# luisdamiano/sparseRGPs

Hardware: AMD Instinct MI355X
Metric: sparse-GP objective+gradient evals/sec at n=1e6, m=1024, d=8 (higher is better)
Workload: dtype f64; 1 GPU; C3: Titsias VI ELBO + gradient, n=1000000, m=1024, d=8, ard, P=10, knots fixed; n=1000000, m=1024, d=8, kernel=ard, parallelism=single

## Files before the change

sparsergps_amd/csrc/capi.hip:

```cpp
#include <math.h>

#include <cmath>
#include <stdarg.h>
#include <stdio.h>
#include <stdlib.h>
#include <string.h>
#include <time.h>

#include <algorithm>
#include <string>
#include <vector>

#include "../../include/sgp.h"
#include "../../include/sgp_diag.h"
#include "sgp_internal.h"

#ifdef SGP_HOST_PROBE
extern "C" __attribute__((visibility("default"))) double sgp_probe_t[4] = {0.0, 0.0, 0.0, 0.0};
#endif
#include "sgp_probe.h"
#include "sgp_multi.h"

namespace {

// ... 246 lines not shown
  bool lap_expo_rows = false;
  const double* lap_av = nullptr;
  int lap_family = SGP_FAM_POISSON;
  std::vector<double> lap_objs;
  bool timing = false;
  std::string timing_only;
  int64_t timing_evals = 0;
  std::vector<Timer> timers;
  std::vector<hipEvent_t> pool;
  size_t pool_used = 0;
};

namespace {

constexpr int SC_LD22 = 0, SC_LDB = 1, SC_TU = 2, SC_TRKS = 3, SC_TRBS = 4, SC_RR = 5,
              SC_G22 = 16;
constexpr int SC_N = 64;
constexpr int SLAB_SMALL = 1024 * (SGP_MAXD + 2);
constexpr int KNOT_PART_ROWS = 256;
constexpr int RB_N = 256;

constexpr int RB_SEGS = SGP_RB_SEGS;

#ifdef SGP_HOST_PROBE
static double hp_now() {
  struct timespec ts;
  clock_gettime(CLOCK_MONOTONIC, &ts);
  return (double)ts.tv_sec + 1e-9 * (double)ts.tv_nsec;
}
static double hp_t0 = 0.0, hp_issue = 0.0, hp_wait = 0.0, hp_tail = 0.0, hp_prev_end = 0.0,
              hp_gap = 0.0;
static long hp_n = 0;
// ... 512 lines not shown
                   hipSuccess && cus > 0)
      c->sk_slots = 2 * cus;
    if (c->sk_slots > 0) {
      st = st ? st : dalloc(&c->sk_ws, sgp_con_sk_doubles(c->sk_slots));
      st = st ? st : dalloc(&c->sk_flags, c->sk_slots + 1);
      if (!st && hipMemset(c->sk_flags, 0, sizeof(unsigned) * (c->sk_slots + 1)) != hipSuccess) {
        set_err("hipMemset of the contraction hand-over flags failed");
        st = SGP_EHIP;
      }
    }
  }
  c->slab_small_cap = std::max<int64_t>(SLAB_SMALL, mp * (SGP_MAXD + 2));
  st = st ? st : dalloc(&c->slab_small, c->slab_small_cap);
  st = st ? st : dalloc(&c->slab_aux, c->slab_small_cap);
  st = st ? st : dalloc(&c->rr_dev, 1);
  st = st ? st : dalloc(&c->mmpart, mp);
  st = st ? st : dalloc(&c->sc, SC_N);
  st = st ? st : dalloc(&c->y, np_);
  st = st ? st : dalloc(&c->mu, np_);
  st = st ? st : dalloc(&c->tslab, (np_ / 64) * mp);
  st = st ? st : dalloc(&c->khash, mp);
  st = st ? st : dalloc(&c->kidx, mp);
  st = st ? st : dalloc(&c->cflag, np_);
  if (!st && (hipHostMalloc(reinterpret_cast<void**>(&c->pin),
                            sizeof(double) * (mp * d + m_max + (m_max + 1) / 2 + 8 + RB_N),
                            hipHostMallocDefault) != hipSuccess ||
              hipEventCreateWithFlags(&c->ev_pin, hipEventDisableTiming) != hipSuccess)) {
    set_err("pinned staging allocation failed");
    st = SGP_ENOMEM;
  }
  if (st) {
// ... 212 lines not shown
  }
  c->pack_red1 = enable != 0;
  return SGP_OK;
}

static int64_t vi_red1_toff(const sgp_ctx* c, int64_t mp) {
  return c->pack_red1 ? syrk_packed_doubles(mp) : mp * mp;
}

int64_t sgp_knot_red_extra(int d, int64_t m) { return round_up(m, SGP_TILE) * d; }

static int contract_pass(sgp_ctx* c, const double* M, ConArgs ca, double* rec_out,
                         double* knot_out, bool knot_acc) {
  int64_t nrec = 0, nwg = 0;
  if (c->knot_on) ca.knot_slab = c->knot_slab;
  const bool fused = ca.uvec != nullptr && ca.alpha_in == nullptr;
  if (fused) ca.alpha_out = c->alpha;
  if (c->sk_ws) {
    if (++c->sk_epoch == 0) ++c->sk_epoch;
    ca.sk_ws = c->sk_ws;
    ca.sk_flags = c->sk_flags;
    ca.sk_epoch = c->sk_epoch;
    ca.sk_slots = c->sk_slots;
    ca.sk_status = c->status + 3;
    ca.sk_dp = con_sk_dp();
  }
  HIPCHK(launch_contract_args(c->kp, c->K, M, c->X, c->n_pad, c->n, c->n_pad, c->U, c->mp, c->m,
                              c->mp, ca, c->slab_con, &nrec, &nwg, c->stream));
  const bool flags_known = c->cflag_gen == c->knots_gen;
  HIPCHK(launch_records(c->slab_con, nrec, nwg, c->X, c->n_pad, c->n, c->kp.d, c->U, c->mp, c->m,
                        c->khash, c->kidx, c->K, c->mp, M, ca, fused ? c->alpha : ca.alpha_in,
                        c->slab_small, c->slab_small_cap, 1 + c->kp.L, rec_out, c->cflag,
                        flags_known ? 2 : 1, c->stream, c->defer_rec ? &c->rec_defer : nullptr));
  c->cflag_gen = c->knots_gen;
  if (c->knot_on)
    HIPCHK(launch_knot_reduce(c->knot_slab, c->n_pad / SGP_TILE, c->mp, c->kp.d, c->knot_part,
                              KNOT_PART_ROWS * c->mp_max * c->d,
                              knot_out, knot_acc, c->stream));
  return SGP_OK;
}

static int knot_finish(sgp_ctx* c, const double* knot_red, const double* uvec, const double* Ainv,
                       const double* Binv, const double* M3, double a, double b, double cc,
                       const double* v, const double* w, double e2) {
  if (!c->knot_on) return SGP_OK;
  const KernParams& kp = c->kp;
// ... 253 lines not shown
    Scope tm(c, "mm_vectors");
    const bool k22_via_t = c->t_deferred;
    if (c->t_deferred) {
      HIPCHK(hipStreamWaitEvent(c->stream, c->ev_t, 0));
      c->t_deferred = false;
    }
    if (flags & SGP_FLAG_OBJ_ONLY) {
      HIPCHK(dense_gemv(c->Binv, mp, t, 1.0 / z, c->uvec, c->stream));
      HIPCHK(launch_dot(t, c->uvec, mp, c->slab_small, c->sc + SC_TU, c->stream));
      HIPCHK(hipMemcpyAsync(c->sc + SC_RR, red1 + toff + mp, sizeof(double),
                            hipMemcpyDeviceToDevice, c->stream));
      HIPCHK(hipStreamWaitEvent(c->stream, c->ev_m3, 0));
      c->phase = 2;
      return SGP_OK;
    }
    if (!k22_via_t) HIPCHK(hipStreamWaitEvent(c->stream, c->ev_k22, 0));
    HIPCHK(launch_vi_mm_rows(c->Binv, c->K22inv, S, t, mp, 1.0 / z, 1.0 / kp.tau2, -1.0 / z,
                             c->uvec, c->Pm, c->mmpart, c->stream));
    HIPCHK(hipEventRecord(c->ev_bm, c->stream));
  }
  {
    HIPCHK(hipStreamWaitEvent(c->aux_lo, c->ev_bm, 0));
    HIPCHK(launch_vi_mm_scalars(t, c->uvec, c->mmpart, mp, red1 + toff + mp, c->sc + SC_TU,
                                c->sc + SC_TRBS, c->sc + SC_RR, c->aux_lo));
    HIPCHK(launch_sum_small(c->logdB, mp / SGP_DB, c->sc + SC_LDB, c->aux_lo));
    Scope tm(c, "contract_kmm", c->aux_lo);
    int nb = 0;
    HIPCHK(launch_contract_kmm(kp, c->U, c->mp, c->m, mp, c->uvec, c->K22inv, c->Binv, c->M3,
                               -0.5, 0.5, -1.0 / (2.0 * kp.tau2), nullptr, nullptr, 0.0,
                               c->slab_aux, c->slab_small_cap, &nb, c->aux_lo));
    HIPCHK(launch_colsum(c->slab_aux, nb, kp.P, c->sc + SC_G22, c->aux_lo));
    HIPCHK(hipEventRecord(c->ev_m3, c->aux_lo));
  }
  {
    Scope tm(c, "contract_knm");
    ConArgs ca;
    ca.r = c->r;
    ca.invz = 1.0 / z;
    ca.uvec = c->uvec;
    ca.cdiag = c->cdiag;
    ca.count_a2 = 1;
    int st2 = contract_pass(c, c->Pm, ca, red2, red2 + sgp_vi_red2_count(kp.kernel, kp.d), false);
    if (st2) return st2;
  }
  HIPCHK(hipStreamWaitEvent(c->stream, c->ev_m3, 0));
  c->phase = 2;
  return SGP_OK;
}

int sgp_vi_finish(sgp_ctx* c, const double* red2, double* obj, double* grad) {
  MULTI_REFUSE(c, "sgp_vi_finish");
  const bool obj_only = c && (c->flags & SGP_FLAG_OBJ_ONLY);
  if (!c || !red2 || !obj || (!grad && !obj_only)) {
    set_err("invalid arguments");
    return SGP_EINVAL;
  }
  if (c->phase != 2) { set_err("sgp_vi_finish called before sgp_vi_phase2"); return SGP_EINVAL; }
  {
    const hipError_t e = hipSetDevice(c->device);
// ... 32 lines not shown
    fprintf(stderr, "\n");
  }
  const double n = (double)c->n_global;
  const double z = kp.tau2 + c->delta;
  const double ld22 = 2.0 * sc[SC_LD22], ldB = 2.0 * sc[SC_LDB];
  const double rr = sc[SC_RR], tu = sc[SC_TU], trKS = sc[SC_TRKS], trBS = sc[SC_TRBS];
  const double quad = -0.5 * rr / z + 0.5 * tu / z;
  const double logdet22 = (c->flags & SGP_FLAG_R_DET) ? log(exp(ld22)) : ld22;
  const double det_part = -0.5 * (n * log(z) - logdet22 + ldB);
  const double trace_term = -(1.0 / (2.0 * kp.tau2)) * (n * (kp.sig2 + c->delta) - trKS);
  *obj = quad + det_part - (n / 2.0) * log(2.0 * M_PI) + trace_term;
  if (obj_only) {
    c->knot_raw.clear();
    return SGP_OK;
  }
  const double e_sig = r2[0];
  const double c_sum = r2[1 + L], c_cnt = r2[2 + L], c_dg = r2[3 + L], aTa = r2[4 + L];
  const double trSinv = n / z - trBS / (z * z);
  const double trW = 0.5 * (aTa - trSinv);
  grad[0] = 2.0 * e_sig + sc[SC_G22] - n * kp.sig2 / kp.tau2;
  for (int q = 0; q < L; ++q) grad[1 + q] = r2[1 + q] + sc[SC_G22 + 1 + q];
  grad[L + 1] = 2.0 * kp.tau2 * (c_sum - (c_cnt - c->delta * c_dg) / kp.tau2) +
                2.0 * kp.tau2 * trW - 2.0 * trace_term;
  return knot_finish(c, red2 + n2, c->uvec, c->K22inv, c->Binv, c->M3, -0.5, 0.5,
                     -1.0 / (2.0 * kp.tau2), nullptr, nullptr, 0.0);
}

int sgp_eval_vi(sgp_ctx* c, int kernel, const double* theta, const double* U, int64_t m,
                int64_t ldu, double delta, unsigned flags, double* obj, double* grad) {
  MULTI_FWD(c, obj && (grad || (flags & SGP_FLAG_OBJ_ONLY)) ? multi_eval_vi(c->multi, kernel, theta, U, m, ldu, delta, flags, obj, grad) : multi_bad_args());
  if (!c) { set_err("context is NULL"); return SGP_EINVAL; }
  if (!obj || (!grad && !(flags & SGP_FLAG_OBJ_ONLY))) {
    set_err("obj is NULL, or grad is NULL without SGP_FLAG_OBJ_ONLY");
    return SGP_EINVAL;
  }
#ifdef SGP_HOST_PROBE
// ... 1430 lines not shown
```

sparsergps_amd/csrc/k_dense.hip:

```cpp
#include <stdlib.h>

#include <atomic>

#include "sgp_internal.h"
#include "sgp_probe.h"

namespace {

__device__ __forceinline__ double wave_sum(double v) {
#pragma unroll
  for (int o = 32; o > 0; o >>= 1) v += __shfl_xor(v, o, 64);
  return v;
}

__device__ __forceinline__ double block_sum(double v, double* sh) {
  const int lane = threadIdx.x & 63, w = threadIdx.x >> 6;
  v = wave_sum(v);
  if (lane == 0) sh[w] = v;
  __syncthreads();
  double t = 0.0;
  const int nw = blockDim.x >> 6;
  for (int q = 0; q < nw; ++q) t += sh[q];
  __syncthreads();
  return t;
// ... 760 lines not shown
                                                    int64_t n_pad, double* __restrict__ omega,
                                                    double* __restrict__ slab) {
  __shared__ double sh[4];
  double s = 0.0;
  for (int64_t i = (int64_t)blockIdx.x * 256 + threadIdx.x; i < n_pad; i += (int64_t)gridDim.x * 256) {
    double o = 0.0;
    if (i < n) o = alpha[i] * alpha[i] - (w[i] - w[i] * w[i] * p[i]);
    omega[i] = o;
    s += o;
  }
  s = block_sum(s, sh);
  if (threadIdx.x == 0) slab[blockIdx.x] = s;
}

__global__ void __launch_bounds__(256) k_vi_mm_rows(const double* __restrict__ Binv,
                                                    const double* __restrict__ K22inv,
                                                    const double* __restrict__ S,
                                                    const double* __restrict__ t, int64_t mp,
                                                    double invz, double a, double b,
                                                    double* __restrict__ u,
                                                    double* __restrict__ P,
                                                    double* __restrict__ part) {
  const int64_t row = (int64_t)blockIdx.x * 4 + (threadIdx.x >> 6);
  const int lane = threadIdx.x & 63;
  if (row >= mp) return;
  const int64_t o = row * mp;
  double su = 0.0, sp = 0.0;
  for (int64_t j = lane; j < mp; j += 64) {
    const double bv = Binv[o + j];
    su = fma(bv, t[j], su);
    sp = fma(bv, S[o + j], sp);
    P[o + j] = a * K22inv[o + j] + b * bv;
  }
  su = wave_sum(su);
  sp = wave_sum(sp);
  if (lane == 0) {
    u[row] = invz * su;
    part[row] = sp;
  }
}

__global__ void __launch_bounds__(256) k_vi_mm_scalars(const double* __restrict__ t,
                                                       const double* __restrict__ u,
                                                       const double* __restrict__ part,
                                                       int64_t mp, const double* __restrict__ rr,
                                                       double* __restrict__ tu_out,
                                                       double* __restrict__ trbs_out,
                                                       double* __restrict__ rr_out) {
  __shared__ double sh[4];
  double a = 0.0, c = 0.0;
  for (int64_t j = threadIdx.x; j < mp; j += 256) {
    a = fma(t[j], u[j], a);
    c += part[j];
  }
  a = block_sum(a, sh);
  c = block_sum(c, sh);
  if (threadIdx.x == 0) {
    *tu_out = a;
    *trbs_out = c;
    *rr_out = *rr;
  }
}

}

hipError_t launch_vi_mm_rows(const double* Binv, const double* K22inv, const double* S,
                             const double* t, int64_t mp, double invz, double a, double b,
                             double* u, double* P, double* part, hipStream_t s) {
  hipLaunchKernelGGL(k_vi_mm_rows, dim3((unsigned)((mp + 3) / 4)), dim3(256), 0, s, Binv, K22inv,
                     S, t, mp, invz, a, b, u, P, part);
  return hipGetLastError();
}

hipError_t launch_vi_mm_scalars(const double* t, const double* u, const double* part, int64_t mp,
                                const double* rr, double* tu_out, double* trbs_out,
                                double* rr_out, hipStream_t s) {
  hipLaunchKernelGGL(k_vi_mm_scalars, dim3(1), dim3(256), 0, s, t, u, part, mp, rr, tu_out,
                     trbs_out, rr_out);
  return hipGetLastError();
}

hipError_t launch_fitc_z(const double* q, int64_t n, int64_t n_pad, double c0, double* w,
                         double* slab, int* nblocks, hipStream_t s) {
  int nb = (int)((n_pad + 255) / 256);
  if (nb > 1024) nb = 1024;
// ... 163 lines not shown
```

sparsergps_amd/csrc/k_mfma.hip:

```cpp
#include <algorithm>
#include <vector>

#include "sgp_internal.h"
#include "sgp_probe.h"

namespace {

constexpr int T128 = 128;
constexpr int BK = 16;
constexpr int SB = 144;
constexpr int SA = 17;
constexpr int SYRK_RGRP = 16;

__device__ __forceinline__ double wave_sum(double v) {
#pragma unroll
  for (int o = 32; o > 0; o >>= 1) v += __shfl_xor(v, o, 64);
  return v;
}

__device__ __forceinline__ int64_t xcd_remap(int64_t orig, int64_t nwg) {
  const int64_t x = orig % 8, q = nwg / 8, r = nwg % 8;
  const int64_t base = (x < r) ? x * (q + 1) : r * (q + 1) + (x - r) * q;
  return base + orig / 8;
}
// ... 763 lines not shown
enum { CON_FULL = 0, CON_TAIL = 1, CON_HEAD = 2 };
constexpr int64_t CON_SK_SLOT = 65 * 256;
struct ConSK {
  double* ws = nullptr;
  int dp = -1;
  unsigned* flags = nullptr;
  unsigned epoch = 0;
  int64_t slot = 0;
  int* status = nullptr;
};

__device__ __forceinline__ unsigned con_ldu_sc1(const unsigned* p) {
  return __hip_atomic_load(p, __ATOMIC_RELAXED, __HIP_MEMORY_SCOPE_AGENT);
}

template <int DT, int EPI, bool V2, bool KNOT, bool FROM_T, bool KU, bool T2, int SKM>
__device__ __forceinline__ void con_tile(
    const KernParams& kp, const double* __restrict__ K, const double* __restrict__ M,
    const double* __restrict__ X, int64_t ldx, int64_t n, int64_t n_pad,
    const double* __restrict__ U, int64_t ldu, int64_t m, int64_t mp, const ConArgs& ca,
    double* __restrict__ slab, int nrec, double* __restrict__ rowq, int64_t ti, int64_t tj,
    int64_t wgid, int kb, int ke, double* lds, double (*red)[SGP_MAXD + 5], double (*s_uk)[BK],
    const ConSK& sk, int part, int tid_in) {
  const double* __restrict__ r = ca.r;
  const double* __restrict__ uvec = ca.uvec;
  const double* __restrict__ cdiag = ca.cdiag;
  constexpr int A_SZ = CON_A_SZ, B_SZ = CON_B_SZ;
  const int64_t ntj = mp / T128;
  const int64_t nwg = (n_pad / T128) * ntj;
  const int64_t i0 = ti * T128, j0 = tj * T128;

  const int tid = tid_in, lane = tid & 63, wv = tid >> 6;
  const int wr = wv >> 1, wc = wv & 1;
  const bool with_u = KU && (uvec != nullptr) && (ca.alpha_in == nullptr);
  constexpr bool with_v = V2;

  d4 acc[4][4];
#pragma unroll
  for (int a = 0; a < 4; ++a)
#pragma unroll
    for (int b = 0; b < 4; ++b) acc[a][b] = d4{0.0, 0.0, 0.0, 0.0};

  const int arow = tid >> 1, acol = (tid & 1) * 8;
  const double2* gA = reinterpret_cast<const double2*>(K + (i0 + arow) * mp + acol);
  const int bk = tid >> 4, bc = tid & 15;
  const double2* gB = reinterpret_cast<const double2*>(M + (int64_t)bk * mp + j0) + bc;
  const int64_t bstep = BK * mp / 2;
  double2 va0, va1, va2, va3, vb0, vb1, vb2, vb3;
  double ku = 0.0, vuk = 0.0;
  const double* __restrict__ uk_src = with_u ? uvec : M;
// ... 121 lines not shown
  SGP_PROBE_CON_SKIP_EPILOGUE()
  double* s_alpha = lds;
  double* s_rs = s_alpha + T128;
  double* s_u = s_rs + T128;
  double* s_cd = s_u + T128;
  double* s_beta = s_cd + T128;
  double* s_v = s_beta + T128;
  double* s_xs = s_v + T128;
  double* s_us = s_xs + T128 * 16;
  double* s_rs2 = lds + 8320;
  static_assert(8320 + T128 <= 2 * (A_SZ + B_SZ), "s_rs2 fits the LDS image");
  ku += __shfl_xor(ku, 1, 64);
  double a2 = 0.0;
  if ((tid & 1) == 0) {
    const int64_t i = i0 + arow;
    const double iz = ca.invz_vec ? ca.invz_vec[i] : ca.invz;
    const double al = ca.alpha_in ? ca.alpha_in[i]
                                  : (with_u ? (r[i] - ku) * iz : 0.0);
    const bool iv = i < n;
    s_alpha[arow] = iv ? al : 0.0;
    s_rs[arow] = iv ? (ca.rs_vec ? ca.rs * ca.rs_vec[i] : ca.rs) : 0.0;
    if constexpr (T2) s_rs2[arow] = iv ? (ca.rs_vec2 ? ca.rs2 * ca.rs_vec2[i] : ca.rs2) : 0.0;
    s_beta[arow] = (with_v && iv) ? ca.beta_in[i] : 0.0;
    if (tj == 0) {
      if (ca.count_a2 && i < n) a2 = al * al;
      if (ca.alpha_out) ca.alpha_out[i] = al;
    }
  }
  const double* Kt = K + i0 * mp + j0;

  if constexpr (EPI == EPI_ROWQUAD) {
    if (ca.tstore != nullptr) {
#pragma unroll
      for (int fm = 0; fm < 4; ++fm)
#pragma unroll
        for (int fn = 0; fn < 4; ++fn)
#pragma unroll
          for (int q = 0; q < 4; ++q)
            ca.tstore[(i0 + wr * 64 + fm * 16 + (lane >> 4) + 4 * q) * mp + j0 + wc * 64 +
                      fn * 16 + (lane & 15)] = acc[fm][fn][q];
    }
// ... 126 lines not shown
          for (int fn = 0; fn < 4; ++fn) {
            const int col = wc * 64 + fn * 16 + (lane & 15);
            double kv[2];
#pragma unroll
            for (int r2 = 0; r2 < 2; ++r2) kv[r2] = kb[(wr * 8 + (lane >> 4) + 4 * r2) * KST + col];
#pragma unroll
            for (int r2 = 0; r2 < 2; ++r2) {
              const int q = 2 * h + r2;
              const int row = wr * 64 + fm * 16 + (lane >> 4) + 4 * q;
              double G = s_rs[row] * acc[fm][fn][q];
              if constexpr (T2) G = fma(s_rs2[row], t2c[r2][fn], G);
              if constexpr (V2) G = fma(s_beta[row], vcol[fn], G);
              G = fma(s_alpha[row], ucol[fn], G);
              double w = G * kv[r2];
              if constexpr ((V2 && KNOT) || FROM_T) w = (j0 + col < m && i0 + row < n) ? w : 0.0;
              Cc[fn] += w;
              acc[fm][fn][q] = w;
            }
          }
#pragma unroll
          for (int r2 = 0; r2 < 2; ++r2)
#pragma unroll
            for (int fn = 0; fn < 4; ++fn)
#ifndef SGP_CON_PROBE_NO_EPI_MFMA
              P[fn] = __builtin_amdgcn_mfma_f64_16x16x4f64(acc[fm][fn][2 * h + r2], xb[r2], P[fn],
                                                           0, 0, 0);
#else
              P[fn][r2] = fma(acc[fm][fn][2 * h + r2], xb[r2], P[fn][r2]);
#endif
          if (hs == 1) SGP_PROBE_CON_STAMP(3);
        }
// ... 18 lines not shown
#pragma unroll
            for (int r4 = 0; r4 < 4; ++r4)
              xb[r4] = s_xs[(wr * 64 + fm * 16 + 4 * r4 + (lane >> 4)) * 16 + (lane & 15)];
#pragma unroll
            for (int r4 = 0; r4 < 4; ++r4)
#pragma unroll
              for (int fn = 0; fn < 4; ++fn)
                P[fn] = __builtin_amdgcn_mfma_f64_16x16x4f64(acc[fm][fn][r4], xb[r4], P[fn], 0,
                                                             0, 0);
          }
        }
        const bool cok = 8 * ch + cc < d;
        double E = 0.0;
#pragma unroll
        for (int fn = 0; fn < 4; ++fn) {
          double C = Cc[fn];
          C += __shfl_xor(C, 16, 64);
          C += __shfl_xor(C, 32, 64);
          if (ch == 0 && (lane >> 4) == 0) e_sig += C;
#pragma unroll
          for (int q = 0; q < 4; ++q) {
            const int jl = wc * 64 + fn * 16 + (lane >> 4) + 4 * q;
            const double Cq = __shfl(C, (lane >> 4) + 4 * q, 64);
            const double u = cok ? s_us[jl * sus + cc] : 0.0;
            const double pv = P[fn][q];
            E += (cp >= 8) ? pv : u * fma(u, Cq, -2.0 * pv);
            if constexpr (KNOT) {
              if (cp < 8) s_kn[(wr * T128 + jl) * 8 + cc] = pv - u * Cq;
            }
          }
        }
        E += __shfl_xor(E, 8, 64);
        E += __shfl_xor(E, 16, 64);
        E += __shfl_xor(E, 32, 64);
        if (ard) {
          if (lane < 8 && 8 * ch + lane < d) red[wv][1 + 8 * ch + lane] = E;
        } else {
          double t = E;
          t += __shfl_xor(t, 1, 64);
          t += __shfl_xor(t, 2, 64);
          t += __shfl_xor(t, 4, 64);
          e_sq += t;
        }
        if constexpr (KNOT) {
          __syncthreads();
          for (int e = tid; e < T128 * 8; e += 256) {
            const int col = e >> 3, c = e & 7, cg = 8 * ch + c;
            if (cg < d)
              ca.knot_slab[(ti * mp + j0 + col) * d + cg] =
                  s_kn[col * 8 + c] + s_kn[(T128 + col) * 8 + c];
          }
        }
      }
#undef CON_XSTAGE
    }

    SGP_PROBE_CON_STAMP(6);
    double v;
    v = wave_sum(e_sig);
    if (lane == 0) red[wv][0] = v;
    if (!ard && lane == 0) red[wv][1] = e_sq * rl2s;
    v = wave_sum(a2);
    if (lane == 0) {
      red[wv][1 + L] = 0.0;
      red[wv][2 + L] = 0.0;
      red[wv][3 + L] = 0.0;
      red[wv][4 + L] = v;
    }
    __syncthreads();
    if (tid < nrec)
      slab[tid * nwg + wgid] = red[0][tid] + red[1][tid] + red[2][tid] + red[3][tid];
    SGP_PROBE_CON_STAMP(2);
  }
  if constexpr (SGP_CON_EPI_PRIO > 0) __builtin_amdgcn_s_setprio(0);
}

template <int DT, int EPI, bool V2 = false, bool KNOT = false, bool FROM_T = false, bool KU = true,
          bool T2 = false>
__global__ void __launch_bounds__(256, 2)
k_contract(KernParams kp, const double* __restrict__ K, const double* __restrict__ M,
           const double* __restrict__ X, int64_t ldx, int64_t n, int64_t n_pad,
           const double* __restrict__ U, int64_t ldu, int64_t m, int64_t mp, ConArgs ca,
           double* __restrict__ slab, int nrec, double* __restrict__ rowq) {
  __shared__ __attribute__((aligned(16))) double lds[CON_LDS];
  __shared__ double red[4][SGP_MAXD + 5];
  __shared__ double s_uk[2][BK];
  const int64_t ntj = mp / T128;
  const int64_t nwg = (n_pad / T128) * ntj;
  const int64_t wgid = xcd_remap(blockIdx.x, nwg);
  con_tile<DT, EPI, V2, KNOT, FROM_T, KU, T2, 0>(
      kp, K, M, X, ldx, n, n_pad, U, ldu, m, mp, ca, slab, nrec, rowq, wgid / ntj, wgid % ntj,
      wgid, 0, (int)(mp / BK), lds, red, s_uk, ConSK{}, CON_FULL, (int)threadIdx.x);
}

template <int DT, bool KNOT>
__global__ void __launch_bounds__(256, 2)
k_contract_sk(KernParams kp, const double* __restrict__ K, const double* __restrict__ M,
              const double* __restrict__ X, int64_t ldx, int64_t n, int64_t n_pad,
              const double* __restrict__ U, int64_t ldu, int64_t m, int64_t mp, ConArgs ca,
              double* __restrict__ slab, int nrec, ConSK sk) {
  __shared__ __attribute__((aligned(16))) double lds[CON_LDS];
  __shared__ double red[4][SGP_MAXD + 5];
  __shared__ double s_uk[2][BK];
  const int64_t ntj = mp / T128;
  const int64_t ntiles = (n_pad / T128) * ntj;
  const int S = (int)(mp / BK);
  const int64_t G = gridDim.x, v = xcd_remap(blockIdx.x, G);
  const int64_t dp_rounds = (sk.dp >= 0 && sk.dp < ntiles / G) ? sk.dp : ntiles / G - 1;
  const int64_t t0 = dp_rounds * G;
  const int64_t Usk = (ntiles - t0) * S;
  const int64_t u1 = Usk * (v + 1) / G;
  int64_t u = Usk * v / G;
  if (u % S != 0) {
    const int64_t tile = t0 + u / S;
    const int kb = (int)(u % S);
    ConSK p = sk;
    p.slot = v;
    con_tile<DT, EPI_GRAD, false, KNOT, false, true, false, CON_TAIL>(
        kp, K, M, X, ldx, n, n_pad, U, ldu, m, mp, ca, slab, nrec, nullptr, tile / ntj,
        tile % ntj, tile, kb, S, lds, red, s_uk, p, CON_TAIL, (int)threadIdx.x);
    u += S - kb;
    __syncthreads();
  }
  int64_t r = 0;
  for (;;) {
    int64_t tile;
    int ke;
    if (r < dp_rounds) {
      tile = r * G + v;
      ke = S;
      ++r;
    } else if (u < u1) {
      tile = t0 + u / S;
      ke = (int)((u1 - u) < (int64_t)S ? (u1 - u) : S);
      u += ke;
    } else {
      break;
    }
    ConSK p = sk;
    p.slot = v + 1;
    int tid;
    asm volatile("v_mov_b32 %0, %1" : "=v"(tid) : "v"((int)threadIdx.x));
    con_tile<DT, EPI_GRAD, false, KNOT, false, true, false, CON_HEAD>(
        kp, K, M, X, ldx, n, n_pad, U, ldu, m, mp, ca, slab, nrec, nullptr, tile / ntj,
        tile % ntj, tile, 0, ke, lds, red, s_uk, p, ke < S ? CON_HEAD : CON_FULL, tid);
    __syncthreads();
  }
}

__global__ void __launch_bounds__(256)
k_knot_reduce1(const double* __restrict__ slab, int64_t ntiles, int64_t ncol,
               double* __restrict__ part) {
  const int64_t col = (int64_t)blockIdx.x * 256 + threadIdx.x;
  const int64_t r = blockIdx.y, G = gridDim.y;
  if (col >= ncol) return;
  double s0 = 0.0, s1 = 0.0, s2 = 0.0, s3 = 0.0;
  int64_t t = r;
  for (; t + 3 * G < ntiles; t += 4 * G) {
// ... 40 lines not shown
      h *= 1099511628211ull;
    }
  }
  return h;
}

struct CoincArgs {
  const double* X; int64_t ldx, n; int d;
  const double* U; int64_t ldu, m;
  const uint64_t* khash; const int* kidx;
  const double* K; int64_t mp; const double* M;
  const double* alpha; const double* uvec; const double* beta; const double* vvec;
  const double* rs_vec; double rs; const double* cdiag;
  uint8_t* cflag; int flag_mode;
  const double* M2; const double* rs_vec2; double rs2;
};

__device__ __forceinline__ void coinc_body(const CoincArgs& ca, int64_t bid, int64_t nblk,
                                           double* __restrict__ part) {
  const double* __restrict__ X = ca.X;
  const double* __restrict__ U = ca.U;
  const double* __restrict__ K = ca.K;
  const double* __restrict__ M = ca.M;
  const int64_t ldx = ca.ldx, n = ca.n, ldu = ca.ldu, m = ca.m, mp = ca.mp;
  const int d = ca.d, flag_mode = ca.flag_mode;
  const uint64_t* __restrict__ khash = ca.khash;
  const int* __restrict__ kidx = ca.kidx;
  const double *alpha = ca.alpha, *uvec = ca.uvec, *beta = ca.beta, *vvec = ca.vvec;
  const double *rs_vec = ca.rs_vec, *cdiag = ca.cdiag;
  const double rs = ca.rs;
// ... 11 lines not shown
    for (int64_t p = lo; p < m && khash[p] == h; ++p) {
      const int64_t j = kidx[p];
      bool eq = true;
      for (int c = 0; c < d; ++c) eq = eq && (X[i + c * ldx] == U[j + c * ldu]);
      if (!eq) continue;
      any = true;
      double t = 0.0;
      for (int64_t k = 0; k < m; ++k) t = fma(K[i * mp + k], M[k * mp + j], t);
      double g = (rs_vec ? rs * rs_vec[i] : rs) * t;
      if (ca.M2) {
        double t2 = 0.0;
        for (int64_t k = 0; k < m; ++k) t2 = fma(K[i * mp + k], ca.M2[k * mp + j], t2);
        g = fma(ca.rs_vec2 ? ca.rs2 * ca.rs_vec2[i] : ca.rs2, t2, g);
      }
      if (beta) g = fma(beta[i], vvec[j], g);
      if (alpha && uvec) g = fma(alpha[i], uvec[j], g);
      a[0] += g;
      a[1] += 1.0;
      a[2] += cdiag ? cdiag[j] : 0.0;
    }
    if (flag_mode == 1) cflag[i] = any ? 1 : 0;
  }
  __shared__ double sh[4][3];
  const int lane = threadIdx.x & 63, w = threadIdx.x >> 6;
  for (int k = 0; k < 3; ++k) {
    const double v = wave_sum(a[k]);
    if (lane == 0) sh[w][k] = v;
  }
  __syncthreads();
  if (threadIdx.x < 3)
    part[bid * 3 + threadIdx.x] =
// ... 507 lines not shown
                          int64_t ldx, int64_t n, int d, const double* U, int64_t ldu, int64_t m,
                          const uint64_t* khash, const int* kidx, const double* K, int64_t mp,
                          const double* M, const ConArgs& cg, const double* alpha, double* part,
                          int64_t part_cap, int coff, double* rec, uint8_t* cflag, int flag_mode,
                          hipStream_t s, RecPass2* defer) {
  if (nrow <= 0 || nrow > 256 || coff < 0 || coff + 3 > nrow) return hipErrorInvalidValue;
  const int G = 32;
  int64_t nbc = (n + 255) / 256;
  if (nbc > 1024) nbc = 1024;
  if (nbc < 1) nbc = 1;
  if (nrow * G + 3 * nbc > part_cap) return hipErrorInvalidValue;
  double* part_r = part;
  double* part_c = part + nrow * G;
  CoincArgs ca{X, ldx, n, d, U, ldu, m, khash, kidx, K, mp, M, alpha, cg.uvec, cg.beta_in,
               cg.vvec, cg.rs_vec, cg.rs, cg.cdiag, cflag, flag_mode, cg.M2, cg.rs_vec2,
               cg.rs2};
  hipLaunchKernelGGL(k_rec_pass1, dim3((unsigned)(nbc + nrow * G)), dim3(256), 0, s, ca,
                     (int)nbc, slab, len, G, part_r, part_c);
  RecPass2 p2;
  p2.part_r = part_r;
  p2.part_c = part_c;
  p2.rec = rec;
  p2.G = G;
  p2.nrow = (int)nrow;
  p2.nbc = (int)nbc;
  p2.coff = coff;
  if (defer != nullptr) *defer = p2;
  else hipLaunchKernelGGL(k_rec_pass2, dim3(1), dim3(256), 0, s, p2);
  return hipGetLastError();
}

// ... 23 lines not shown
}

template <int DT, bool KNOT = false>
static void launch_con_grad(bool v2, const KernParams& kp, const double* K, const double* M,
                            const double* X, int64_t ldx, int64_t n, int64_t n_pad,
                            const double* U, int64_t ldu, int64_t m, int64_t mp,
                            const ConArgs& ca, double* slab, int nrec, int64_t nwg,
                            hipStream_t s) {
  if (!v2 && con_use_sk(ca, nwg, mp)) {
    ConSK sk;
    sk.ws = ca.sk_ws;
    sk.flags = ca.sk_flags;
    sk.epoch = ca.sk_epoch;
    sk.status = ca.sk_status;
    sk.dp = ca.sk_dp;
    hipLaunchKernelGGL((k_contract_sk<DT, KNOT>), dim3((unsigned)ca.sk_slots), dim3(256), 0, s,
                       kp, K, M, X, ldx, n, n_pad, U, ldu, m, mp, ca, slab, nrec, sk);
    return;
  }
  if (v2)
    hipLaunchKernelGGL((k_contract<DT, EPI_GRAD, true, KNOT>), dim3((unsigned)nwg), dim3(256), SGP_CON_SHMEM,
                       s, kp, K, M, X, ldx, n, n_pad, U, ldu, m, mp, ca, slab, nrec,
                       (double*)nullptr);
  else
    hipLaunchKernelGGL((k_contract<DT, EPI_GRAD, false, KNOT>), dim3((unsigned)nwg), dim3(256), SGP_CON_SHMEM,
                       s, kp, K, M, X, ldx, n, n_pad, U, ldu, m, mp, ca, slab, nrec,
                       (double*)nullptr);
}

template <int DT, bool T2>
static void launch_con_from_t2(bool v2, bool kn, const KernParams& kp, const double* K,
                               const double* M, const double* X, int64_t ldx, int64_t n,
                               int64_t n_pad, const double* U, int64_t ldu, int64_t m, int64_t mp,
                               const ConArgs& ca, double* slab, int nrec, int64_t nwg,
                               hipStream_t s) {
// ... 29 lines not shown
                                  nrec, nwg, s);
}

int64_t sgp_con_sk_doubles(int slots) { return (int64_t)(slots + 1) * CON_SK_SLOT; }

hipError_t launch_contract_args(const KernParams& kp, const double* K, const double* M,
                                const double* X, int64_t ldx, int64_t n, int64_t n_pad,
                                const double* U, int64_t ldu, int64_t m, int64_t mp,
                                const ConArgs& ca, double* slab, int64_t* nrec_out,
                                int64_t* nwg_out, hipStream_t s) {
  const int64_t nwg = (n_pad / T128) * (mp / T128);
  const int nrec = kp.L + 5;
  *nrec_out = nrec;
  *nwg_out = nwg;
  if ((ca.tin2 != nullptr) != (ca.M2 != nullptr) || (ca.tin2 && (!ca.tin || kp.d > 8)))
    return hipErrorInvalidValue;
  if (ca.tin != nullptr) {
    if (ca.uvec != nullptr && ca.alpha_in == nullptr) return hipErrorInvalidValue;
    const bool v2 = ca.beta_in != nullptr, kn = ca.knot_slab != nullptr;
    if (kp.d <= 8) launch_con_from_t<8>(v2, kn, kp, K, M, X, ldx, n, n_pad, U, ldu, m, mp, ca, slab,
                                        nrec, nwg, s);
    else launch_con_from_t<SGP_MAXD>(v2, kn, kp, K, M, X, ldx, n, n_pad, U, ldu, m, mp, ca, slab,
                                     nrec, nwg, s);
    return hipGetLastError();
  }
  if (ca.knot_slab != nullptr) {
    const bool v2 = ca.beta_in != nullptr;
    if (kp.d <= 8) launch_con_grad<8, true>(v2, kp, K, M, X, ldx, n, n_pad, U, ldu, m, mp, ca,
                                            slab, nrec, nwg, s);
    else launch_con_grad<SGP_MAXD, true>(v2, kp, K, M, X, ldx, n, n_pad, U, ldu, m, mp, ca, slab,
// ... 81 lines not shown
```

sparsergps_amd/csrc/sgp_internal.h:

```cpp
#pragma once
#include <hip/hip_runtime.h>
#include <stdint.h>

#define SGP_MAXD 32
#define SGP_TILE 128
#define SGP_DB 64
#define SGP_GJ_SYNC_WORDS (128 + 2 * 64 * 64)

typedef double d4 __attribute__((ext_vector_type(4)));

__device__ __forceinline__ double sgp_exp_nonpos(double x) {
  constexpr double c2 = 1.0 / 2, c3 = 1.0 / 6, c4 = 1.0 / 24, c5 = 1.0 / 120, c6 = 1.0 / 720,
                   c7 = 1.0 / 5040, c8 = 1.0 / 40320, c9 = 1.0 / 362880, c10 = 1.0 / 3628800,
                   c11 = 1.0 / 39916800, c12 = 1.0 / 479001600, c13 = 1.0 / 6227020800.0;
  const double k = __builtin_rint(x * 1.4426950408889634074);
  double r = __builtin_fma(-k, 6.93147180369123816490e-01, x);
  r = __builtin_fma(-k, 1.90821492927058770002e-10, r);
  double p = c13;
  p = __builtin_fma(p, r, c12);
  p = __builtin_fma(p, r, c11);
  p = __builtin_fma(p, r, c10);
  p = __builtin_fma(p, r, c9);
  p = __builtin_fma(p, r, c8);
  p = __builtin_fma(p, r, c7);
// ... 99 lines not shown
int64_t syrk_slab_doubles(int64_t n_pad, int64_t mp);
bool syrk_use_s256(int64_t mp, bool with_t);
struct ConArgs {
  const double* r = nullptr;
  double invz = 0.0;
  const double* invz_vec = nullptr;
  const double* uvec = nullptr;
  const double* alpha_in = nullptr;
  const double* beta_in = nullptr;
  const double* vvec = nullptr;
  const double* rs_vec = nullptr;
  double rs = 1.0;
  const double* cdiag = nullptr;
  int count_a2 = 0;
  double* alpha_out = nullptr;
  double* knot_slab = nullptr;
  double* tstore = nullptr;
  const double* tin = nullptr;
  const double* tin2 = nullptr;
  const double* M2 = nullptr;
  const double* rs_vec2 = nullptr;
  double rs2 = 0.0;
  double* sk_ws = nullptr;
  unsigned* sk_flags = nullptr;
  unsigned sk_epoch = 0;
  int sk_slots = 0;
  int* sk_status = nullptr;
  int sk_dp = -1;
};
int64_t sgp_con_sk_doubles(int slots);
// ... 20 lines not shown
                         hipStream_t s);

hipError_t dense_spd_inverse(double* A, int64_t mp, double* R, double* P, double* logd,
                             int* status, unsigned* sync, hipStream_t s);
hipError_t dense_spd_inverse_sum(const double* A0, double beta, const double* B0, double* out,
                                 int64_t mp, double* R, double* P, double* logd, int* status,
                                 unsigned* sync, hipStream_t s);
hipError_t dense_spd_inverse_chain(double* A, int64_t mp, double* R, double* P, double* logd,
                                   int* status, unsigned* sync, hipStream_t s, bool per_step);
hipError_t dense_spd_inverse_sum_chain(const double* A0, double beta, const double* B0,
                                       double* out, int64_t mp, double* R, double* P, double* logd,
                                       int* status, unsigned* sync, hipStream_t s, bool per_step);
hipError_t dense_axpby(double a, const double* A, double b, const double* B, double* C,
                       int64_t count, hipStream_t s);
hipError_t launch_vi_mm_rows(const double* Binv, const double* K22inv, const double* S,
                             const double* t, int64_t mp, double invz, double a, double b,
                             double* u, double* P, double* part, hipStream_t s);
hipError_t launch_vi_mm_scalars(const double* t, const double* u, const double* part, int64_t mp,
                                const double* rr, double* tu_out, double* trbs_out,
                                double* rr_out, hipStream_t s);
hipError_t dense_gemv(const double* A, int64_t mp, const double* x, double scale, double* y,
                      hipStream_t s);
hipError_t launch_dot(const double* a, const double* b, int64_t count, double* partial,
                      double* out, hipStream_t s);
hipError_t launch_colsum(const double* slab, int64_t nrows, int64_t ncol, double* out,
                         hipStream_t s);
hipError_t launch_diag(const double* A, int64_t mp, int64_t lda, double* out, hipStream_t s);
hipError_t launch_sum_small(const double* v, int64_t count, double* out, hipStream_t s);
hipError_t launch_sum_and_diag(const double* v, int64_t count, double* sum, const double* A,
                               int64_t mp, int64_t lda, double* diag, hipStream_t s);

hipError_t launch_fitc_z(const double* q, int64_t n, int64_t n_pad, double c0, double* w,
                         double* slab, int* nblocks, hipStream_t s);
hipError_t launch_fitc_omega(const double* alpha, const double* w, const double* p, int64_t n,
                             int64_t n_pad, double* omega, double* slab, int* nblocks,
// ... 87 lines not shown
```

Before: 20.63 evals/s.

## Fold the u-dependent VI gradient terms out of the n-sized contraction into m-sized kernels

The rank-one u·uᵀ correction is folded into the Pm matrix, and the large K_nm contraction uses alpha = r/z directly, so it no longer has to compute K·u per row or accumulate the column sums. The terms lost this way (the e_sig, lengthscale and aTa corrections) are rebuilt on the side stream by new column-fold and scalar kernels over the m×m S and P matrices. The aim is to remove per-element work and the epilogue column reduction from the dominant n×m pass, at the cost of extra O(m²) kernels and a separate gemv to form u.

```diff
diff --git a/sparsergps_amd/csrc/capi.hip b/sparsergps_amd/csrc/capi.hip
--- a/sparsergps_amd/csrc/capi.hip
+++ b/sparsergps_amd/csrc/capi.hip
@@ -284,8 +284,11 @@
 namespace {
 
 constexpr int SC_LD22 = 0, SC_LDB = 1, SC_TU = 2, SC_TRKS = 3, SC_TRBS = 4, SC_RR = 5,
-              SC_G22 = 16;
-constexpr int SC_N = 64;
+              SC_ESIG = 6, SC_ATA = 7,
+              SC_G22 = 16,
+              SC_EL = 64;
+constexpr int SC_N = 96;
+static_assert(SC_G22 + SGP_MAXD + 2 <= SC_EL && SC_EL + SGP_MAXD <= SC_N, "sc slots overlap");
 constexpr int SLAB_SMALL = 1024 * (SGP_MAXD + 2);
 constexpr int KNOT_PART_ROWS = 256;
 constexpr int RB_N = 256;
@@ -828,7 +831,7 @@
   st = st ? st : dalloc(&c->slab_small, c->slab_small_cap);
   st = st ? st : dalloc(&c->slab_aux, c->slab_small_cap);
   st = st ? st : dalloc(&c->rr_dev, 1);
-  st = st ? st : dalloc(&c->mmpart, mp);
+  st = st ? st : dalloc(&c->mmpart, 3 * mp);
   st = st ? st : dalloc(&c->sc, SC_N);
   st = st ? st : dalloc(&c->y, np_);
   st = st ? st : dalloc(&c->mu, np_);
@@ -1071,7 +1074,7 @@
                          double* knot_out, bool knot_acc) {
   int64_t nrec = 0, nwg = 0;
   if (c->knot_on) ca.knot_slab = c->knot_slab;
-  const bool fused = ca.uvec != nullptr && ca.alpha_in == nullptr;
+  const bool fused = ca.uvec != nullptr && ca.alpha_in == nullptr && !ca.vi_fold;
   if (fused) ca.alpha_out = c->alpha;
   if (c->sk_ws) {
     if (++c->sk_epoch == 0) ++c->sk_epoch;
@@ -1086,7 +1089,8 @@
                               c->mp, ca, c->slab_con, &nrec, &nwg, c->stream));
   const bool flags_known = c->cflag_gen == c->knots_gen;
   HIPCHK(launch_records(c->slab_con, nrec, nwg, c->X, c->n_pad, c->n, c->kp.d, c->U, c->mp, c->m,
-                        c->khash, c->kidx, c->K, c->mp, M, ca, fused ? c->alpha : ca.alpha_in,
+                        c->khash, c->kidx, c->K, c->mp, M, ca,
+                        ca.vi_fold ? ca.r : (fused ? c->alpha : ca.alpha_in),
                         c->slab_small, c->slab_small_cap, 1 + c->kp.L, rec_out, c->cflag,
                         flags_known ? 2 : 1, c->stream, c->defer_rec ? &c->rec_defer : nullptr));
   c->cflag_gen = c->knots_gen;
@@ -1370,9 +1374,10 @@
       c->phase = 2;
       return SGP_OK;
     }
+    HIPCHK(dense_gemv(c->Binv, mp, t, 1.0 / z, c->uvec, c->stream));
     if (!k22_via_t) HIPCHK(hipStreamWaitEvent(c->stream, c->ev_k22, 0));
-    HIPCHK(launch_vi_mm_rows(c->Binv, c->K22inv, S, t, mp, 1.0 / z, 1.0 / kp.tau2, -1.0 / z,
-                             c->uvec, c->Pm, c->mmpart, c->stream));
+    HIPCHK(launch_vi_mm_rows(c->Binv, c->K22inv, S, c->uvec, mp, 1.0 / kp.tau2, -1.0 / z,
+                             -1.0 / z, c->Pm, c->mmpart, c->stream));
     HIPCHK(hipEventRecord(c->ev_bm, c->stream));
   }
   {
@@ -1386,8 +1391,8 @@
                                -0.5, 0.5, -1.0 / (2.0 * kp.tau2), nullptr, nullptr, 0.0,
                                c->slab_aux, c->slab_small_cap, &nb, c->aux_lo));
     HIPCHK(launch_colsum(c->slab_aux, nb, kp.P, c->sc + SC_G22, c->aux_lo));
-    HIPCHK(hipEventRecord(c->ev_m3, c->aux_lo));
-  }
+  }
+  int st2 = SGP_OK;
   {
     Scope tm(c, "contract_knm");
     ConArgs ca;
@@ -1395,10 +1400,15 @@
     ca.invz = 1.0 / z;
     ca.uvec = c->uvec;
     ca.cdiag = c->cdiag;
-    ca.count_a2 = 1;
-    int st2 = contract_pass(c, c->Pm, ca, red2, red2 + sgp_vi_red2_count(kp.kernel, kp.d), false);
-    if (st2) return st2;
-  }
+    ca.vi_fold = true;
+    st2 = contract_pass(c, c->Pm, ca, red2, red2 + sgp_vi_red2_count(kp.kernel, kp.d), false);
+  }
+  if (!st2)
+    HIPCHK(launch_vi_fold_cols(kp, S, c->Pm, t, c->uvec, c->U, c->mp, c->m, mp, 1.0 / z,
+                               red1 + toff + mp, c->mmpart + mp, !c->knot_on, c->sc + SC_ESIG,
+                               c->sc + SC_EL, c->sc + SC_ATA, c->aux_lo));
+  HIPCHK(hipEventRecord(c->ev_m3, c->aux_lo));
+  if (st2) return st2;
   HIPCHK(hipStreamWaitEvent(c->stream, c->ev_m3, 0));
   c->phase = 2;
   return SGP_OK;
@@ -1461,12 +1471,13 @@
     c->knot_raw.clear();
     return SGP_OK;
   }
-  const double e_sig = r2[0];
-  const double c_sum = r2[1 + L], c_cnt = r2[2 + L], c_dg = r2[3 + L], aTa = r2[4 + L];
+  const double e_sig = r2[0] + sc[SC_ESIG];
+  const double c_sum = r2[1 + L], c_cnt = r2[2 + L], c_dg = r2[3 + L];
+  const double aTa = r2[4 + L] + sc[SC_ATA];
   const double trSinv = n / z - trBS / (z * z);
   const double trW = 0.5 * (aTa - trSinv);
   grad[0] = 2.0 * e_sig + sc[SC_G22] - n * kp.sig2 / kp.tau2;
-  for (int q = 0; q < L; ++q) grad[1 + q] = r2[1 + q] + sc[SC_G22 + 1 + q];
+  for (int q = 0; q < L; ++q) grad[1 + q] = r2[1 + q] + sc[SC_EL + q] + sc[SC_G22 + 1 + q];
   grad[L + 1] = 2.0 * kp.tau2 * (c_sum - (c_cnt - c->delta * c_dg) / kp.tau2) +
                 2.0 * kp.tau2 * trW - 2.0 * trace_term;
   return knot_finish(c, red2 + n2, c->uvec, c->K22inv, c->Binv, c->M3, -0.5, 0.5,
diff --git a/sparsergps_amd/csrc/k_dense.hip b/sparsergps_amd/csrc/k_dense.hip
--- a/sparsergps_amd/csrc/k_dense.hip
+++ b/sparsergps_amd/csrc/k_dense.hip
@@ -798,30 +798,96 @@
 }
 
 __global__ void __launch_bounds__(256) k_vi_mm_rows(const double* __restrict__ Binv,
-                                                    const double* __restrict__ K22inv,
-                                                    const double* __restrict__ S,
-                                                    const double* __restrict__ t, int64_t mp,
-                                                    double invz, double a, double b,
-                                                    double* __restrict__ u,
-                                                    double* __restrict__ P,
-                                                    double* __restrict__ part) {
+                                                         const double* __restrict__ K22inv,
+                                                         const double* __restrict__ S,
+                                                         const double* __restrict__ u, int64_t mp,
+                                                         double a, double b, double c1,
+                                                         double* __restrict__ P,
+                                                         double* __restrict__ part) {
   const int64_t row = (int64_t)blockIdx.x * 4 + (threadIdx.x >> 6);
   const int lane = threadIdx.x & 63;
   if (row >= mp) return;
   const int64_t o = row * mp;
-  double su = 0.0, sp = 0.0;
+  const double cu = c1 * u[row];
+  double sp = 0.0;
   for (int64_t j = lane; j < mp; j += 64) {
     const double bv = Binv[o + j];
-    su = fma(bv, t[j], su);
     sp = fma(bv, S[o + j], sp);
-    P[o + j] = a * K22inv[o + j] + b * bv;
-  }
-  su = wave_sum(su);
+    P[o + j] = fma(cu, u[j], a * K22inv[o + j] + b * bv);
+  }
   sp = wave_sum(sp);
-  if (lane == 0) {
-    u[row] = invz * su;
-    part[row] = sp;
-  }
+  if (lane == 0) part[row] = sp;
+}
+
+__global__ void __launch_bounds__(256) k_vi_fold_cols(const double* __restrict__ S,
+                                                      const double* __restrict__ P,
+                                                      const double* __restrict__ u, int64_t mp,
+                                                      double* __restrict__ cs) {
+  __shared__ double sh[2][4][64];
+  const int tx = threadIdx.x & 63, ty = threadIdx.x >> 6;
+  const int64_t j = (int64_t)blockIdx.x * 64 + tx;
+  double sp = 0.0, su = 0.0;
+  if (j < mp) {
+    for (int64_t k = ty; k < mp; k += 4) {
+      const double sv = S[k * mp + j];
+      sp = fma(sv, P[k * mp + j], sp);
+      su = fma(sv, u[k], su);
+    }
+  }
+  sh[0][ty][tx] = sp;
+  sh[1][ty][tx] = su;
+  __syncthreads();
+  if (ty == 0 && j < mp) {
+    cs[j] = (sh[0][0][tx] + sh[0][1][tx]) + (sh[0][2][tx] + sh[0][3][tx]);
+    cs[mp + j] = (sh[1][0][tx] + sh[1][1][tx]) + (sh[1][2][tx] + sh[1][3][tx]);
+  }
+}
+
+__global__ void __launch_bounds__(256) k_vi_fold_scalars(KernParams kp, const double* __restrict__ cs,
+                                                         const double* __restrict__ t,
+                                                         const double* __restrict__ u,
+                                                         const double* __restrict__ U, int64_t ldu,
+                                                         int64_t m, int64_t mp, double invz,
+                                                         const double* __restrict__ rr,
+                                                         int col_terms,
+                                                         double* __restrict__ esig_out,
+                                                         double* __restrict__ el_out,
+                                                         double* __restrict__ ata_out) {
+  __shared__ double sh[4];
+  const bool ard = kp.kernel == 1;
+  const int d = kp.d;
+  double e = 0.0, tu = 0.0, usu = 0.0, esq = 0.0;
+  for (int64_t j = threadIdx.x; j < m; j += 256) {
+    const double c = fma(u[j] * invz, t[j], cs[j]);
+    e += c;
+    tu = fma(u[j], t[j], tu);
+    usu = fma(u[j], cs[mp + j], usu);
+    if (!ard && col_terms)
+      for (int q = 0; q < d; ++q) {
+        const double uv = U[j + q * ldu];
+        esq = fma(uv * uv, c, esq);
+      }
+  }
+  e = block_sum(e, sh);
+  tu = block_sum(tu, sh);
+  usu = block_sum(usu, sh);
+  if (threadIdx.x == 0) *ata_out = (*rr - 2.0 * tu + usu) * invz * invz;
+  if (!col_terms) return;
+  if (ard) {
+    for (int q = 0; q < d; ++q) {
+      double v = 0.0;
+      for (int64_t j = threadIdx.x; j < m; j += 256) {
+        const double uv = U[j + q * ldu] * kp.rl[q];
+        v = fma(uv * uv, fma(u[j] * invz, t[j], cs[j]), v);
+      }
+      v = block_sum(v, sh);
+      if (threadIdx.x == 0) el_out[q] = v;
+    }
+  } else {
+    esq = block_sum(esq, sh);
+    if (threadIdx.x == 0) el_out[0] = esq * kp.rl2[0];
+  }
+  if (threadIdx.x == 0) *esig_out = e;
 }
 
 __global__ void __launch_bounds__(256) k_vi_mm_scalars(const double* __restrict__ t,
@@ -849,10 +915,22 @@
 }
 
 hipError_t launch_vi_mm_rows(const double* Binv, const double* K22inv, const double* S,
-                             const double* t, int64_t mp, double invz, double a, double b,
-                             double* u, double* P, double* part, hipStream_t s) {
-  hipLaunchKernelGGL(k_vi_mm_rows, dim3((unsigned)((mp + 3) / 4)), dim3(256), 0, s, Binv, K22inv,
-                     S, t, mp, invz, a, b, u, P, part);
+                                  const double* u, int64_t mp, double a, double b, double c1,
+                                  double* P, double* part, hipStream_t s) {
+  hipLaunchKernelGGL(k_vi_mm_rows, dim3((unsigned)((mp + 3) / 4)), dim3(256), 0, s, Binv,
+                     K22inv, S, u, mp, a, b, c1, P, part);
+  return hipGetLastError();
+}
+
+hipError_t launch_vi_fold_cols(const KernParams& kp, const double* S, const double* P,
+                               const double* t, const double* u, const double* U, int64_t ldu,
+                               int64_t m, int64_t mp, double invz, const double* rr, double* cs,
+                               bool col_terms, double* esig_out, double* el_out,
+                               double* ata_out, hipStream_t s) {
+  hipLaunchKernelGGL(k_vi_fold_cols, dim3((unsigned)((mp + 63) / 64)), dim3(256), 0, s, S, P, u,
+                     mp, cs);
+  hipLaunchKernelGGL(k_vi_fold_scalars, dim3(1), dim3(256), 0, s, kp, cs, t, u, U, ldu, m, mp,
+                     invz, rr, col_terms ? 1 : 0, esig_out, el_out, ata_out);
   return hipGetLastError();
 }
 
diff --git a/sparsergps_amd/csrc/k_mfma.hip b/sparsergps_amd/csrc/k_mfma.hip
--- a/sparsergps_amd/csrc/k_mfma.hip
+++ b/sparsergps_amd/csrc/k_mfma.hip
@@ -801,7 +801,8 @@
   return __hip_atomic_load(p, __ATOMIC_RELAXED, __HIP_MEMORY_SCOPE_AGENT);
 }
 
-template <int DT, int EPI, bool V2, bool KNOT, bool FROM_T, bool KU, bool T2, int SKM>
+template <int DT, int EPI, bool V2, bool KNOT, bool FROM_T, bool KU, bool T2, int SKM,
+          bool VIF = false>
 __device__ __forceinline__ void con_tile(
     const KernParams& kp, const double* __restrict__ K, const double* __restrict__ M,
     const double* __restrict__ X, int64_t ldx, int64_t n, int64_t n_pad,
@@ -821,6 +822,7 @@
   const int wr = wv >> 1, wc = wv & 1;
   const bool with_u = KU && (uvec != nullptr) && (ca.alpha_in == nullptr);
   constexpr bool with_v = V2;
+  constexpr bool NOCS = VIF && !KNOT;
 
   d4 acc[4][4];
 #pragma unroll
@@ -972,17 +974,25 @@
   double a2 = 0.0;
   if ((tid & 1) == 0) {
     const int64_t i = i0 + arow;
-    const double iz = ca.invz_vec ? ca.invz_vec[i] : ca.invz;
-    const double al = ca.alpha_in ? ca.alpha_in[i]
-                                  : (with_u ? (r[i] - ku) * iz : 0.0);
+    double iz, al;
+    if constexpr (VIF) {
+      iz = ca.invz;
+      al = r[i] * iz;
+    } else {
+      iz = ca.invz_vec ? ca.invz_vec[i] : ca.invz;
+      al = ca.alpha_in ? ca.alpha_in[i]
+                       : (with_u ? (r[i] - ku) * iz : 0.0);
+    }
     const bool iv = i < n;
     s_alpha[arow] = iv ? al : 0.0;
     s_rs[arow] = iv ? (ca.rs_vec ? ca.rs * ca.rs_vec[i] : ca.rs) : 0.0;
     if constexpr (T2) s_rs2[arow] = iv ? (ca.rs_vec2 ? ca.rs2 * ca.rs_vec2[i] : ca.rs2) : 0.0;
     s_beta[arow] = (with_v && iv) ? ca.beta_in[i] : 0.0;
-    if (tj == 0) {
-      if (ca.count_a2 && i < n) a2 = al * al;
-      if (ca.alpha_out) ca.alpha_out[i] = al;
+    if constexpr (!VIF) {
+      if (tj == 0) {
+        if (ca.count_a2 && i < n) a2 = al * al;
+        if (ca.alpha_out) ca.alpha_out[i] = al;
+      }
     }
   }
   const double* Kt = K + i0 * mp + j0;
@@ -1139,7 +1149,7 @@
               G = fma(s_alpha[row], ucol[fn], G);
               double w = G * kv[r2];
               if constexpr ((V2 && KNOT) || FROM_T) w = (j0 + col < m && i0 + row < n) ? w : 0.0;
-              Cc[fn] += w;
+              if constexpr (!NOCS) Cc[fn] += w;
               acc[fm][fn][q] = w;
             }
           }
@@ -1188,6 +1198,15 @@
         double E = 0.0;
 #pragma unroll
         for (int fn = 0; fn < 4; ++fn) {
+          if constexpr (NOCS) {
+#pragma unroll
+            for (int q = 0; q < 4; ++q) {
+              const int jl = wc * 64 + fn * 16 + (lane >> 4) + 4 * q;
+              const double u = cok ? s_us[jl * sus + cc] : 0.0;
+              const double pv = P[fn][q];
+              E += (cp >= 8) ? pv : -2.0 * (u * pv);
+            }
+          } else {
           double C = Cc[fn];
           C += __shfl_xor(C, 16, 64);
           C += __shfl_xor(C, 32, 64);
@@ -1202,6 +1221,7 @@
             if constexpr (KNOT) {
               if (cp < 8) s_kn[(wr * T128 + jl) * 8 + cc] = pv - u * Cq;
             }
+          }
           }
         }
         E += __shfl_xor(E, 8, 64);
@@ -1230,11 +1250,12 @@
     }
 
     SGP_PROBE_CON_STAMP(6);
-    double v;
-    v = wave_sum(e_sig);
+    double v = 0.0;
+    if constexpr (!NOCS) v = wave_sum(e_sig);
     if (lane == 0) red[wv][0] = v;
     if (!ard && lane == 0) red[wv][1] = e_sq * rl2s;
-    v = wave_sum(a2);
+    v = 0.0;
+    if constexpr (!VIF) v = wave_sum(a2);
     if (lane == 0) {
       red[wv][1 + L] = 0.0;
       red[wv][2 + L] = 0.0;
@@ -1250,7 +1271,7 @@
 }
 
 template <int DT, int EPI, bool V2 = false, bool KNOT = false, bool FROM_T = false, bool KU = true,
-          bool T2 = false>
+          bool T2 = false, bool VIF = false>
 __global__ void __launch_bounds__(256, 2)
 k_contract(KernParams kp, const double* __restrict__ K, const double* __restrict__ M,
            const double* __restrict__ X, int64_t ldx, int64_t n, int64_t n_pad,
@@ -1262,12 +1283,12 @@
   const int64_t ntj = mp / T128;
   const int64_t nwg = (n_pad / T128) * ntj;
   const int64_t wgid = xcd_remap(blockIdx.x, nwg);
-  con_tile<DT, EPI, V2, KNOT, FROM_T, KU, T2, 0>(
+  con_tile<DT, EPI, V2, KNOT, FROM_T, KU, T2, 0, VIF>(
       kp, K, M, X, ldx, n, n_pad, U, ldu, m, mp, ca, slab, nrec, rowq, wgid / ntj, wgid % ntj,
       wgid, 0, (int)(mp / BK), lds, red, s_uk, ConSK{}, CON_FULL, (int)threadIdx.x);
 }
 
-template <int DT, bool KNOT>
+template <int DT, bool KNOT, bool VIF = false>
 __global__ void __launch_bounds__(256, 2)
 k_contract_sk(KernParams kp, const double* __restrict__ K, const double* __restrict__ M,
               const double* __restrict__ X, int64_t ldx, int64_t n, int64_t n_pad,
@@ -1290,7 +1311,7 @@
     const int kb = (int)(u % S);
     ConSK p = sk;
     p.slot = v;
-    con_tile<DT, EPI_GRAD, false, KNOT, false, true, false, CON_TAIL>(
+    con_tile<DT, EPI_GRAD, false, KNOT, false, !VIF, false, CON_TAIL, VIF>(
         kp, K, M, X, ldx, n, n_pad, U, ldu, m, mp, ca, slab, nrec, nullptr, tile / ntj,
         tile % ntj, tile, kb, S, lds, red, s_uk, p, CON_TAIL, (int)threadIdx.x);
     u += S - kb;
@@ -1315,7 +1336,7 @@
     p.slot = v + 1;
     int tid;
     asm volatile("v_mov_b32 %0, %1" : "=v"(tid) : "v"((int)threadIdx.x));
-    con_tile<DT, EPI_GRAD, false, KNOT, false, true, false, CON_HEAD>(
+    con_tile<DT, EPI_GRAD, false, KNOT, false, !VIF, false, CON_HEAD, VIF>(
         kp, K, M, X, ldx, n, n_pad, U, ldu, m, mp, ca, slab, nrec, nullptr, tile / ntj,
         tile % ntj, tile, 0, ke, lds, red, s_uk, p, ke < S ? CON_HEAD : CON_FULL, tid);
     __syncthreads();
@@ -1386,6 +1407,7 @@
   const double* rs_vec; double rs; const double* cdiag;
   uint8_t* cflag; int flag_mode;
   const double* M2; const double* rs_vec2; double rs2;
+  double ascale;
 };
 
 __device__ __forceinline__ void coinc_body(const CoincArgs& ca, int64_t bid, int64_t nblk,
@@ -1427,7 +1449,7 @@
         g = fma(ca.rs_vec2 ? ca.rs2 * ca.rs_vec2[i] : ca.rs2, t2, g);
       }
       if (beta) g = fma(beta[i], vvec[j], g);
-      if (alpha && uvec) g = fma(alpha[i], uvec[j], g);
+      if (alpha && uvec) g = fma(alpha[i] * ca.ascale, uvec[j], g);
       a[0] += g;
       a[1] += 1.0;
       a[2] += cdiag ? cdiag[j] : 0.0;
@@ -1965,7 +1987,7 @@
   double* part_c = part + nrow * G;
   CoincArgs ca{X, ldx, n, d, U, ldu, m, khash, kidx, K, mp, M, alpha, cg.uvec, cg.beta_in,
                cg.vvec, cg.rs_vec, cg.rs, cg.cdiag, cflag, flag_mode, cg.M2, cg.rs_vec2,
-               cg.rs2};
+               cg.rs2, cg.vi_fold ? cg.invz : 1.0};
   hipLaunchKernelGGL(k_rec_pass1, dim3((unsigned)(nbc + nrow * G)), dim3(256), 0, s, ca,
                      (int)nbc, slab, len, G, part_r, part_c);
   RecPass2 p2;
@@ -2019,11 +2041,19 @@
     sk.epoch = ca.sk_epoch;
     sk.status = ca.sk_status;
     sk.dp = ca.sk_dp;
+    if (ca.vi_fold)
+      hipLaunchKernelGGL((k_contract_sk<DT, KNOT, true>), dim3((unsigned)ca.sk_slots), dim3(256),
+                         0, s, kp, K, M, X, ldx, n, n_pad, U, ldu, m, mp, ca, slab, nrec, sk);
+    else
     hipLaunchKernelGGL((k_contract_sk<DT, KNOT>), dim3((unsigned)ca.sk_slots), dim3(256), 0, s,
                        kp, K, M, X, ldx, n, n_pad, U, ldu, m, mp, ca, slab, nrec, sk);
     return;
   }
-  if (v2)
+  if (ca.vi_fold)
+    hipLaunchKernelGGL((k_contract<DT, EPI_GRAD, false, KNOT, false, false, false, true>),
+                       dim3((unsigned)nwg), dim3(256), SGP_CON_SHMEM, s, kp, K, M, X, ldx, n,
+                       n_pad, U, ldu, m, mp, ca, slab, nrec, (double*)nullptr);
+  else if (v2)
     hipLaunchKernelGGL((k_contract<DT, EPI_GRAD, true, KNOT>), dim3((unsigned)nwg), dim3(256), SGP_CON_SHMEM,
                        s, kp, K, M, X, ldx, n, n_pad, U, ldu, m, mp, ca, slab, nrec,
                        (double*)nullptr);
@@ -2083,6 +2113,8 @@
   *nrec_out = nrec;
   *nwg_out = nwg;
   if ((ca.tin2 != nullptr) != (ca.M2 != nullptr) || (ca.tin2 && (!ca.tin || kp.d > 8)))
+    return hipErrorInvalidValue;
+  if (ca.vi_fold && (ca.tin || ca.beta_in || ca.alpha_in || ca.invz_vec || !ca.uvec || !ca.r))
     return hipErrorInvalidValue;
   if (ca.tin != nullptr) {
     if (ca.uvec != nullptr && ca.alpha_in == nullptr) return hipErrorInvalidValue;
diff --git a/sparsergps_amd/csrc/sgp_internal.h b/sparsergps_amd/csrc/sgp_internal.h
--- a/sparsergps_amd/csrc/sgp_internal.h
+++ b/sparsergps_amd/csrc/sgp_internal.h
@@ -137,6 +137,7 @@
   const double* cdiag = nullptr;
   int count_a2 = 0;
   double* alpha_out = nullptr;
+  bool vi_fold = false;
   double* knot_slab = nullptr;
   double* tstore = nullptr;
   const double* tin = nullptr;
@@ -187,11 +188,16 @@
 hipError_t dense_axpby(double a, const double* A, double b, const double* B, double* C,
                        int64_t count, hipStream_t s);
 hipError_t launch_vi_mm_rows(const double* Binv, const double* K22inv, const double* S,
-                             const double* t, int64_t mp, double invz, double a, double b,
-                             double* u, double* P, double* part, hipStream_t s);
+                             const double* u, int64_t mp, double a, double b, double c1,
+                             double* P, double* part, hipStream_t s);
 hipError_t launch_vi_mm_scalars(const double* t, const double* u, const double* part, int64_t mp,
                                 const double* rr, double* tu_out, double* trbs_out,
                                 double* rr_out, hipStream_t s);
+hipError_t launch_vi_fold_cols(const KernParams& kp, const double* S, const double* P,
+                               const double* t, const double* u, const double* U, int64_t ldu,
+                               int64_t m, int64_t mp, double invz, const double* rr, double* cs,
+                               bool col_terms, double* esig_out, double* el_out,
+                               double* ata_out, hipStream_t s);
 hipError_t dense_gemv(const double* A, int64_t mp, const double* x, double scale, double* y,
                       hipStream_t s);
 hipError_t launch_dot(const double* a, const double* b, int64_t count, double* partial,
```

New measurement: 21.13 evals/s, median of 6. 2.4% higher.
